# aik2mlj/polyffusion

Measured on AMD Instinct MI355X. Metric: denoising steps/sec (8-bar prmat2c, batch 16), higher is better.
Workload: dtype bf16x3; 1 GPU; sdf_chd8bar cond generation, batch 16 per GPU, 1000-step DDPM sampler loop body (BASELINE.json configs[1]); weights: deterministic synthetic, 41.08M params; global_batch=16, parallelism=batch-shard x1

## Files before the change

include/pfhip.h:

```cpp
#ifndef PFHIP_H
#define PFHIP_H

#include <stddef.h>
#include <stdint.h>

#ifdef __cplusplus
extern "C" {
#endif

#define PF_OK 0
#define PF_EINVAL (-1)
#define PF_ENOTFOUND (-2)
#define PF_ESTATE (-3)
#define PF_EHIP (-4)

int pf_version(void);
const char* pf_last_error(void);

typedef struct pf_unet pf_unet;

typedef struct pf_unet_cfg {
  int32_t in_channels, out_channels, channels, n_res_blocks;
  int32_t n_attention_levels;
  int32_t attention_levels[8];
// ... 110 lines not shown

size_t pf_packed_gemm_weight_floats(int n, int k, int taps);
int pf_pack_gemm_weight(const float* w, int n, int k, int taps, float* dst);
int pf_pack_gemm_weight_bf16x3(const float* w, int n, int k, int taps, void* dst);
int pf_pack_upfold_weight_bf16x3(const float* w, int n, int k, void* dst);
size_t pf_wino_weight_bytes(int n, int k);
int pf_pack_wino_weight_bf16x3(const float* w, int n, int k, void* dst);

int pf_gn_scale_shift(const float* x0, int c0, const float* x1, int c1, int batch, int hw, int groups, float eps,
                      const float* gamma, const float* beta, float* scale, float* shift,
                      void* scratch, size_t scratch_bytes, void* stream);
int pf_ln_stats(const float* x, int rows, int c, float eps, float* mean, float* rstd, void* stream);
int pf_ln_planes(const float* x, int rows, int c, float eps, const float* gamma, const float* beta, void* planes, void* stream);
int pf_mlp_geglu_fused(const float* x, int batch, int l, const float* ln_gamma, const float* ln_beta, float ln_eps,
                       const void* w1_bf16x3, const float* b1, const void* w2_bf16x3, const float* b2,
                       float* out, void* out_planes, void* stream);
int pf_mlp_geglu_proj_fused(const float* x, int batch, int l, const float* ln_gamma, const float* ln_beta, float ln_eps,
                            const void* w1_bf16x3, const float* b1, const void* w2_bf16x3, const float* b2,
                            const void* w3_bf16x3, const float* b3, const float* res3, float* out, float* stats3, void* stream);
typedef struct pf_conv_args {
  const float* x0; int32_t c0; const float* x1; int32_t c1;
  int32_t batch, hin, win;
  int32_t ks, stride, ups;
  const float* w; int32_t n;
  int32_t prologue; const float* sc; const float* sh; const float* mean; const float* rstd;
  const float* bias; const float* sbias; int32_t ld_sbias; const float* res; int32_t ld_res;
  int32_t geglu;
  float* out; int32_t ld_out;
  int32_t precision;
  float* stats_out;
  void* splitk_ws; size_t splitk_ws_bytes;
  int32_t a_planes;
  void* out_planes;
  void* qkv_planes;
  int32_t ups_fold;
  const float* skip_x0; int32_t skip_c0;
  const float* skip_x1; int32_t skip_c1;
  const void* skip_w;
  const float* skip_bias;
  const float* gn_stats0; int32_t gn_tiles0;
  const float* gn_stats1; int32_t gn_tiles1;
  const float* gn_gamma; const float* gn_beta;
  float gn_eps; int32_t gn_groups;
  const int64_t* sbias_rows; int32_t sbias_nrows;
  int32_t no_t16;
  int32_t no_pp;
  int32_t force_tile, force_ksplit;
  int32_t x1_bmod;
  const void* w_wino; int32_t wino;
  void* absmax_slot;
} pf_conv_args;
size_t pf_conv_splitk_ws_bytes(const pf_conv_args* a);
int pf_conv_stats_tiles(const pf_conv_args* a);
int pf_gn_finalize_tiles(const float* stats0, int tiles0, int c0, const float* stats1, int tiles1, int c1, int batch, int hw,
                         int groups, float eps, const float* gamma, const float* beta, float* scale, float* shift, void* stream);
int pf_conv2d(const pf_conv_args* a, void* stream);

int pf_attention_bf16x3(const void* qkv_planes, float* o, int ldo, void* o_planes, int batch, int n_heads, int l, int form ,
                        void* stream);
size_t pf_attention_split_scratch_bytes(int batch, int n_heads, int l);
int pf_attention_bf16x3_split(const void* qkv_planes, float* o, int ldo, void* o_planes, int batch, int n_heads, int l, void* scratch, size_t scratch_bytes,
                              void* stream);
int pf_attention(const float* q, int ldq, const float* k, int ldk, const float* v, int ldv, float* o, int ldo,
                 int batch, int n_heads, int d_head, int lq, int lk, void* stream);

typedef struct pf_ddpm pf_ddpm;
typedef struct pf_ddpm_cfg {
  int32_t image_channels, n_channels, n_levels;
  int32_t ch_mults[8];
  int32_t is_attn[8];
  int32_t n_blocks;
  int32_t img_h, img_w;
} pf_ddpm_cfg;
int pf_ddpm_create(const pf_ddpm_cfg* cfg, pf_ddpm** out);
void pf_ddpm_destroy(pf_ddpm* u);
size_t pf_ddpm_weight_bytes(const pf_ddpm* u);
int pf_ddpm_n_params(const pf_ddpm* u);
int pf_ddpm_param_info(const pf_ddpm* u, int i, char* key_buf, size_t key_buf_len, int64_t shape[4], int* ndim);
int pf_ddpm_pack_param(pf_ddpm* u, const char* key, const float* src, const int64_t* shape, int ndim, void* host_blob);
int pf_ddpm_pack_missing(const pf_ddpm* u, char* buf, size_t buf_len);
int pf_ddpm_bind_weights(pf_ddpm* u, const void* dev_blob);
int pf_ddpm_set_precision(pf_ddpm* u, int precision);
int pf_ddpm_get_precision(const pf_ddpm* u);
size_t pf_ddpm_workspace_bytes(const pf_ddpm* u, int batch);
int pf_ddpm_n_launches(const pf_ddpm* u, int batch);
double pf_ddpm_flops(const pf_ddpm* u, int batch);
int pf_ddpm_forward(pf_ddpm* u, const float* x, const int64_t* t, int batch, float* eps, void* workspace, size_t workspace_bytes, void* stream);

size_t pf_attention_wide_scratch_bytes(int batch, int l);
int pf_attention_wide(const float* q, const float* k, const float* v, int ld, float* o, int ldo, int batch, int l, int d, void* scratch,
                      size_t scratch_bytes, void* stream);
size_t pf_convt_weight_floats(int cin, int cout);
int pf_pack_convt_weight_bf16x3(const float* w, int cin, int cout, void* dst);
int pf_pack_convt_weight_f32(const float* w, int cin, int cout, float* dst);
int pf_conv_transpose_f32(const float* x, int batch, int h, int w, int cin, const float* w_packed, int cout, const float* bias, float* out,
                          void* stream);


#ifdef __cplusplus
}
#endif
#endif
```

polyffusion_amd/_lib.py:

```python
from __future__ import annotations

import ctypes as C
import os
from typing import Optional

HERE = os.path.dirname(os.path.abspath(__file__))
X3_VARIANT = {"": "", "bf16": "", "f16": "f16"}.get(os.environ.get("PF_X3", ""), None)
if X3_VARIANT is None:
    raise RuntimeError(f"PF_X3={os.environ['PF_X3']!r}: expected 'bf16' (default) or 'f16'")


def lib_path(variant: str = "") -> str:
    return os.path.join(HERE, f"libpfhip_{variant}.so" if variant else "libpfhip.so")


LIB_PATH = lib_path(X3_VARIANT)
X3_WEIGHT_SCALE = 256.0 if X3_VARIANT == "f16" else 1.0


def x3_torch_dtype(variant: Optional[str] = None):
    import torch
    return torch.float16 if (X3_VARIANT if variant is None else variant) == "f16" else torch.bfloat16


# ... 92 lines not shown
    "pf_unet_track_absmax": (C.c_int, [C.c_void_p, C.c_void_p]),
    "pf_unet_profile_read_direct": (C.c_int, [C.c_void_p, C.POINTER(C.c_double), C.c_int]),
    "pf_unet_profile_read": (C.c_int, [C.c_void_p, C.POINTER(C.c_int), c_float_p, C.POINTER(C.c_double), C.c_int]),
    "pf_unet_n_launches": (C.c_int, [C.c_void_p, C.c_int, C.c_int]),
    "pf_cfg_combine": (C.c_int, [C.c_void_p, C.c_float, C.c_void_p, C.c_size_t, C.c_void_p]),
    "pf_ddpm_step": (C.c_int, [C.c_void_p] * 6 + [C.POINTER(DdpmCoef), C.c_void_p, C.c_size_t, C.c_void_p]),
    "pf_axpby": (C.c_int, [C.c_void_p, C.c_void_p, C.c_float, C.c_float, C.c_void_p, C.c_size_t, C.c_void_p]),
    "pf_ddim_step": (C.c_int, [C.c_void_p] * 6 + [C.POINTER(DdimCoef), C.c_void_p, C.c_size_t, C.c_void_p]),
    "pf_randn": (C.c_int, [C.c_void_p, C.c_size_t, C.c_uint64, C.c_uint64, C.c_uint64, C.c_void_p]),
    "pf_ddpm_step_rng": (C.c_int, [C.c_void_p] * 4 + [C.POINTER(DdpmCoef), C.c_uint64, C.c_uint64, C.c_uint64, C.c_uint64, C.c_void_p, C.c_size_t, C.c_void_p]),
    "pf_ddim_step_rng": (C.c_int, [C.c_void_p] * 5 + [C.POINTER(DdimCoef), C.c_uint64, C.c_uint64, C.c_uint64, C.c_void_p, C.c_size_t, C.c_void_p]),
    "pf_ddpm_step_rng_dev": (C.c_int, [C.c_void_p] * 6 + [C.c_uint64, C.c_uint64, C.c_void_p, C.c_size_t, C.c_void_p]),
    "pf_ddim_step_rng_dev": (C.c_int, [C.c_void_p] * 7 + [C.c_uint64, C.c_uint64, C.c_void_p, C.c_size_t, C.c_void_p]),
    "pf_clock_probe": (C.c_int, [C.c_void_p, C.c_void_p]),
    "pf_mfma_probe": (C.c_int, [C.c_void_p, C.c_int, C.POINTER(C.c_double), C.c_void_p]),
    "pf_step_state_set": (C.c_int, [C.c_void_p, C.c_int64, C.c_uint64, C.c_void_p]),
    "pf_step_begin": (C.c_int, [C.c_void_p, C.c_void_p, C.c_void_p, C.c_int, C.c_void_p]),
    "pf_step_end": (C.c_int, [C.c_void_p, C.c_int, C.c_void_p]),
    "pf_randn_dev": (C.c_int, [C.c_void_p, C.c_size_t, C.c_uint64, C.c_void_p, C.c_int, C.c_uint64, C.c_void_p]),
    "pf_ddpm_step_dev": (C.c_int, [C.c_void_p] * 6 + [C.c_void_p, C.c_void_p, C.c_void_p, C.c_size_t, C.c_void_p]),
    "pf_ddim_step_dev": (C.c_int, [C.c_void_p] * 6 + [C.c_void_p, C.c_void_p, C.c_void_p, C.c_size_t, C.c_void_p]),
    "pf_comm_unique_id": (C.c_int, [C.c_void_p]),
    "pf_comm_init": (C.c_int, [C.c_void_p, C.c_int, C.c_int, C.POINTER(C.c_void_p)]),
    "pf_comm_bcast": (C.c_int, [C.c_void_p, C.c_void_p, C.c_size_t, C.c_int, C.c_void_p]),
    "pf_comm_destroy": (C.c_int, [C.c_void_p]),
    "pf_prmat2c_durations": (C.c_int, [C.c_void_p, C.c_int, C.c_int, C.c_int, C.c_void_p, C.c_void_p]),
    "pf_encoder_create": (C.c_int, [C.c_int] * 6 + [C.POINTER(C.c_void_p)]),
    "pf_encoder_destroy": (None, [C.c_void_p]),
    "pf_encoder_weight_bytes": (C.c_size_t, [C.c_void_p]),
    "pf_encoder_pack_param": (C.c_int, [C.c_void_p, C.c_char_p, C.c_void_p, c_i64_p, C.c_int, C.c_void_p]),
    "pf_encoder_pack_missing": (C.c_int, [C.c_void_p, C.c_char_p, C.c_size_t]),
    "pf_encoder_bind_weights": (C.c_int, [C.c_void_p, C.c_void_p]),
    "pf_encoder_workspace_bytes": (C.c_size_t, [C.c_void_p, C.c_int]),
    "pf_encoder_forward": (C.c_int, [C.c_void_p, C.c_void_p, C.c_int, C.c_int, C.c_void_p, C.c_void_p, C.c_size_t, C.c_void_p]),
    "pf_packed_gemm_weight_floats": (C.c_size_t, [C.c_int, C.c_int, C.c_int]),
    "pf_pack_gemm_weight": (C.c_int, [C.c_void_p, C.c_int, C.c_int, C.c_int, C.c_void_p]),
    "pf_pack_gemm_weight_bf16x3": (C.c_int, [C.c_void_p, C.c_int, C.c_int, C.c_int, C.c_void_p]),
    "pf_pack_upfold_weight_bf16x3": (C.c_int, [C.c_void_p, C.c_int, C.c_int, C.c_void_p]),
    "pf_wino_weight_bytes": (C.c_size_t, [C.c_int, C.c_int]),
    "pf_pack_wino_weight_bf16x3": (C.c_int, [C.c_void_p, C.c_int, C.c_int, C.c_void_p]),
    "pf_unet_set_precision": (C.c_int, [C.c_void_p, C.c_int]),
    "pf_unet_get_precision": (C.c_int, [C.c_void_p]),
    "pf_x3_element": (C.c_int, []),
    "pf_gn_scale_shift": (C.c_int, [C.c_void_p, C.c_int, C.c_void_p, C.c_int, C.c_int, C.c_int, C.c_int, C.c_float,
                                    C.c_void_p, C.c_void_p, C.c_void_p, C.c_void_p, C.c_void_p, C.c_size_t, C.c_void_p]),
    "pf_ln_stats": (C.c_int, [C.c_void_p, C.c_int, C.c_int, C.c_float, C.c_void_p, C.c_void_p, C.c_void_p]),
    "pf_ln_planes": (C.c_int, [C.c_void_p, C.c_int, C.c_int, C.c_float, C.c_void_p, C.c_void_p, C.c_void_p, C.c_void_p]),
    "pf_mlp_geglu_fused": (C.c_int, [C.c_void_p, C.c_int, C.c_int, C.c_void_p, C.c_void_p, C.c_float, C.c_void_p, C.c_void_p, C.c_void_p,
                                     C.c_void_p, C.c_void_p, C.c_void_p, C.c_void_p]),
    "pf_mlp_geglu_proj_fused": (C.c_int, [C.c_void_p, C.c_int, C.c_int, C.c_void_p, C.c_void_p, C.c_float] + [C.c_void_p] * 10),
    "pf_conv2d": (C.c_int, [C.POINTER(ConvArgs), C.c_void_p]),
    "pf_conv_stats_tiles": (C.c_int, [C.POINTER(ConvArgs)]),
    "pf_conv_splitk_ws_bytes": (C.c_size_t, [C.POINTER(ConvArgs)]),
    "pf_gn_finalize_tiles": (C.c_int, [C.c_void_p, C.c_int, C.c_int, C.c_void_p, C.c_int, C.c_int, C.c_int, C.c_int, C.c_int,
                                       C.c_float, C.c_void_p, C.c_void_p, C.c_void_p, C.c_void_p, C.c_void_p]),
    "pf_attention_bf16x3": (C.c_int, [C.c_void_p, C.c_void_p, C.c_int, C.c_void_p, C.c_int, C.c_int, C.c_int, C.c_int, C.c_void_p]),
    "pf_attention_split_scratch_bytes": (C.c_size_t, [C.c_int, C.c_int, C.c_int]),
    "pf_attention_bf16x3_split": (C.c_int, [C.c_void_p, C.c_void_p, C.c_int, C.c_void_p, C.c_int, C.c_int, C.c_int, C.c_void_p, C.c_size_t, C.c_void_p]),
    "pf_attention": (C.c_int, [C.c_void_p, C.c_int, C.c_void_p, C.c_int, C.c_void_p, C.c_int, C.c_void_p, C.c_int,
                               C.c_int, C.c_int, C.c_int, C.c_int, C.c_int, C.c_void_p]),
    "pf_ddpm_create": (C.c_int, [C.POINTER(DDPMCfg), C.POINTER(C.c_void_p)]),
    "pf_ddpm_destroy": (None, [C.c_void_p]),
    "pf_ddpm_weight_bytes": (C.c_size_t, [C.c_void_p]),
    "pf_ddpm_n_params": (C.c_int, [C.c_void_p]),
    "pf_ddpm_param_info": (C.c_int, [C.c_void_p, C.c_int, C.c_char_p, C.c_size_t, c_i64_p, C.POINTER(C.c_int)]),
    "pf_ddpm_pack_param": (C.c_int, [C.c_void_p, C.c_char_p, C.c_void_p, c_i64_p, C.c_int, C.c_void_p]),
    "pf_ddpm_pack_missing": (C.c_int, [C.c_void_p, C.c_char_p, C.c_size_t]),
    "pf_ddpm_bind_weights": (C.c_int, [C.c_void_p, C.c_void_p]),
    "pf_ddpm_set_precision": (C.c_int, [C.c_void_p, C.c_int]),
    "pf_ddpm_get_precision": (C.c_int, [C.c_void_p]),
    "pf_ddpm_workspace_bytes": (C.c_size_t, [C.c_void_p, C.c_int]),
    "pf_ddpm_n_launches": (C.c_int, [C.c_void_p, C.c_int]),
    "pf_ddpm_flops": (C.c_double, [C.c_void_p, C.c_int]),
    "pf_ddpm_forward": (C.c_int, [C.c_void_p, C.c_void_p, C.c_void_p, C.c_int, C.c_void_p, C.c_void_p, C.c_size_t, C.c_void_p]),
    "pf_attention_wide_scratch_bytes": (C.c_size_t, [C.c_int, C.c_int]),
    "pf_attention_wide": (C.c_int, [C.c_void_p, C.c_void_p, C.c_void_p, C.c_int, C.c_void_p, C.c_int, C.c_int, C.c_int, C.c_int,
                                    C.c_void_p, C.c_size_t, C.c_void_p]),
    "pf_convt_weight_floats": (C.c_size_t, [C.c_int, C.c_int]),
    "pf_pack_convt_weight_bf16x3": (C.c_int, [C.c_void_p, C.c_int, C.c_int, C.c_void_p]),
    "pf_pack_convt_weight_f32": (C.c_int, [C.c_void_p, C.c_int, C.c_int, C.c_void_p]),
    "pf_conv_transpose_f32": (C.c_int, [C.c_void_p, C.c_int, C.c_int, C.c_int, C.c_int, C.c_void_p, C.c_int, C.c_void_p, C.c_void_p,
                                        C.c_void_p]),
}

_libs: dict = {}


def load(variant: Optional[str] = None) -> C.CDLL:
    v = X3_VARIANT if variant is None else variant
    if v in _libs:
        return _libs[v]
    path = lib_path(v)
    if not os.path.exists(path):
        raise RuntimeError(
            f"{path} not found: the HIP extension is not built. Run `python -m polyffusion_amd.build{' --variant=' + v if v else ''}` "
            "(or __graft_entry__.build()). There is no CPU fallback for this path.")
    lib = C.CDLL(path, mode=os.RTLD_LOCAL | os.RTLD_NOW)
    for name, (res, args) in SIGNATURES.items():
        fn = getattr(lib, name)
        fn.restype = res
        fn.argtypes = args
    if lib.pf_x3_element() != (1 if v == "f16" else 0):
        raise RuntimeError(f"{path}: built with the wrong split element type (pf_x3_element() = {lib.pf_x3_element()})")
    _libs[v] = lib
    return lib

# ... 22 lines not shown
```

polyffusion_amd/build.py:

```python
from __future__ import annotations

import os
import subprocess
import sys

HERE = os.path.dirname(os.path.abspath(__file__))
CSRC = os.path.join(HERE, "csrc")
SOURCES = ["conv_mfma.hip", "conv_bf16x3.hip", "conv_wino.hip", "gemm_planes_bf3.hip", "mlp_fused_bf3.hip", "attention.hip", "attention_bf3.hip", "norm_stats.hip", "small_kernels.hip", "encoders.hip", "comm.hip", "plan.hip", "unet_blocks.hip", "unet.hip", "attention_wide.hip", "ddpm_unet.hip", "abi_ops.hip"]
LIB = os.path.join(HERE, "libpfhip.so")
VARIANTS = {"": [], "f16": ["-DPF_X3_F16"]}


def lib_path(variant: str = "") -> str:
    return os.path.join(HERE, f"libpfhip_{variant}.so" if variant else "libpfhip.so")
HIPCC = os.environ.get("HIPCC", "/opt/rocm/bin/hipcc")
FLAGS = ["--offload-arch=gfx950", "-O3", "-std=c++17", "-fPIC", "-Wall", "-Wno-unused-function"] + (["-DPF_TRACE"] if os.environ.get("PF_TRACE") else [])
EXTRA_FLAGS = {"attention_bf3.hip": ["-fno-slp-vectorize"]}


STAMP = os.path.join(CSRC, ".build_stamp.json")


def _digest(paths, extra=()) -> str:
    import hashlib
    h = hashlib.sha256()
    for p in paths:
        with open(p, "rb") as f:
            h.update(hashlib.sha256(f.read()).digest())
    for e in extra:
        h.update(str(e).encode())
        h.update(b"\0")
    return h.hexdigest()


def _read_stamp() -> dict:
    import json
    try:
        with open(STAMP) as f:
            return json.load(f)
    except (OSError, ValueError):
        return {}


def _write_stamp(st: dict) -> None:
    import json
    with open(STAMP + ".new", "w") as f:
        json.dump(st, f, indent=1, sort_keys=True)
    os.replace(STAMP + ".new", STAMP)


def build(force: bool = False, verbose: bool = True, variant: str = "") -> str:
    return build_all(force, verbose, (variant,))[0]


_SLOW_FIRST = ["conv_bf16x3.hip", "conv_wino.hip", "attention_bf3.hip", "mlp_fused_bf3.hip", "conv_mfma.hip", "gemm_planes_bf3.hip"]


def build_all(force: bool = False, verbose: bool = True, variants=("", "f16")) -> list:
    force = force or os.environ.get("PF_FORCE_BUILD", "") not in ("", "0")
    hdrs = [os.path.join(CSRC, h) for h in sorted(os.listdir(CSRC)) if h.endswith(".h")] + [os.path.join(HERE, "..", "include", "pfhip.h")]
    stamp = _read_stamp()
# ... 49 lines not shown
```

polyffusion_amd/csrc/abi_ops.hip:

```cpp
#include <stdarg.h>
#include <vector>
#include "plan.h"

namespace pf {

static thread_local std::string g_err;
int set_error(int code, const char* fmt, ...) {
  char buf[512];
  va_list ap;
  va_start(ap, fmt);
  vsnprintf(buf, sizeof buf, fmt, ap);
  va_end(ap);
  g_err = buf;
  return code;
}

}

using namespace pf;

extern "C" {

int pf_version(void) { return 100; }
const char* pf_last_error(void) { return g_err.c_str(); }
// ... 9 lines not shown
int pf_pack_gemm_weight(const float* w, int n, int k, int taps, float* dst) {
  PF_REQUIRE(w && dst && n > 0 && k > 0 && k % 4 == 0 && (taps == 1 || taps == 9), "pf_pack_gemm_weight: bad arguments");
  memset(dst, 0, gemm_floats(taps, k, n) * sizeof(float));
  pack_gemm(dst, w, n, k, taps, (n + 63) / 64 * 64, 0);
  return PF_OK;
}

int pf_pack_gemm_weight_bf16x3(const float* w, int n, int k, int taps, void* dst) {
  PF_REQUIRE(w && dst && n > 0 && k > 0 && k % 8 == 0 && (taps == 1 || taps == 9), "pf_pack_gemm_weight_bf16x3: bad arguments");
  memset(dst, 0, gemm_floats(taps, k, n) * sizeof(float));
  PF_REQUIRE(pack_gemm_bf3(dst, w, n, k, taps, (n + 63) / 64 * 64, 0, nullptr), X3_RANGE_MSG, "pf_pack_gemm_weight_bf16x3");
  return PF_OK;
}

int pf_gn_scale_shift(const float* x0, int c0, const float* x1, int c1, int batch, int hw, int groups, float eps,
                      const float* gamma, const float* beta, float* scale, float* shift, void* scratch, size_t scratch_bytes,
                      void* stream) {
  return launch_gn_scale_shift(x0, c0, x1, c1, batch, hw, groups, eps, gamma, beta, scale, shift, scratch, scratch_bytes, (hipStream_t)stream);
}
int pf_pack_upfold_weight_bf16x3(const float* w, int n, int k, void* dst) {
  PF_REQUIRE(w && dst && n > 0 && k > 0 && k % 8 == 0, "pack_upfold: bad arguments");
  PF_REQUIRE(pack_upfold_bf3(dst, w, n, k, (n + 63) / 64 * 64), X3_RANGE_MSG, "pf_pack_upfold_weight_bf16x3");
  return PF_OK;
}
size_t pf_wino_weight_bytes(int n, int k) { return (n > 0 && k > 0) ? (size_t)16 * k * n * 4 : 0; }
int pf_pack_wino_weight_bf16x3(const float* w, int n, int k, void* dst) {
  PF_REQUIRE(w && dst && n > 0 && k > 0 && n % 64 == 0 && k % 16 == 0, "pack_wino: n must be a multiple of 64 and k of 16 (n=%d k=%d)", n, k);
  PF_REQUIRE(pack_wino_bf3(dst, w, n, k), X3_RANGE_MSG, "pf_pack_wino_weight_bf16x3");
  return PF_OK;
}
int pf_prmat2c_durations(const float* prmat2c, int n, int steps, int custom_round, int32_t* dur, void* stream) {
  return launch_prmat2c_durations(prmat2c, n, steps, custom_round, dur, (hipStream_t)stream);
}
int pf_mlp_geglu_fused(const float* x, int batch, int l, const float* ln_gamma, const float* ln_beta, float ln_eps,
                       const void* w1_bf16x3, const float* b1, const void* w2_bf16x3, const float* b2,
                       float* out, void* out_planes, void* stream) {
  return launch_mlp_fused(x, batch, l, ln_gamma, ln_beta, ln_eps, w1_bf16x3, b1, w2_bf16x3, b2, out, out_planes, (hipStream_t)stream);
}
int pf_mlp_geglu_proj_fused(const float* x, int batch, int l, const float* ln_gamma, const float* ln_beta, float ln_eps,
                            const void* w1_bf16x3, const float* b1, const void* w2_bf16x3, const float* b2,
                            const void* w3_bf16x3, const float* b3, const float* res3, float* out, float* stats3, void* stream) {
  if (!w3_bf16x3) return set_error(PF_EINVAL, "pf_mlp_geglu_proj_fused: null projection weight");
  return launch_mlp_fused(x, batch, l, ln_gamma, ln_beta, ln_eps, w1_bf16x3, b1, w2_bf16x3, b2, out, nullptr, (hipStream_t)stream, w3_bf16x3, b3,
                          res3, stats3);
}
int pf_ln_planes(const float* x, int rows, int c, float eps, const float* gamma, const float* beta, void* planes, void* stream) {
  return launch_ln_planes(x, rows, c, eps, gamma, beta, planes, (hipStream_t)stream);
}
int pf_ln_stats(const float* x, int rows, int c, float eps, float* mean, float* rstd, void* stream) {
  return launch_ln_stats(x, rows, c, eps, mean, rstd, (hipStream_t)stream);
}
int pf_conv_stats_tiles(const pf_conv_args* a) { return a ? conv_stats_tiles(*a) : 0; }
size_t pf_conv_splitk_ws_bytes(const pf_conv_args* a) { return a ? conv_splitk_ws_bytes(*a) : 0; }
int pf_gn_finalize_tiles(const float* stats0, int tiles0, int c0, const float* stats1, int tiles1, int c1, int batch, int hw,
                         int groups, float eps, const float* gamma, const float* beta, float* scale, float* shift, void* stream) {
  return launch_gn_finalize_tiles(stats0, tiles0, c0, stats1, tiles1, c1, batch, hw, groups, eps, gamma, beta, scale, shift,
                                  (hipStream_t)stream);
}
int pf_conv2d(const pf_conv_args* a, void* stream) {
  PF_REQUIRE(a, "pf_conv2d: null argument");
  return launch_conv(*a, (hipStream_t)stream);
}
size_t pf_attention_split_scratch_bytes(int batch, int n_heads, int l) {
  return (batch > 0 && n_heads > 0 && l > 0) ? attention_bf3_split_floats(batch, n_heads, l, nullptr) * sizeof(float) : 0;
}
int pf_attention_bf16x3_split(const void* qkv_planes, float* o, int ldo, void* o_planes, int batch, int n_heads, int l, void* scratch, size_t scratch_bytes,
                              void* stream) {
  return launch_attention_bf3(qkv_planes, o, ldo, o_planes, batch, n_heads, l, 0, (hipStream_t)stream, static_cast<float*>(scratch), scratch_bytes / sizeof(float));
}
int pf_attention_bf16x3(const void* qkv_planes, float* o, int ldo, void* o_planes, int batch, int n_heads, int l, int form, void* stream) {
  return launch_attention_bf3(qkv_planes, o, ldo, o_planes, batch, n_heads, l, form, (hipStream_t)stream);
}
int pf_attention(const float* q, int ldq, const float* k, int ldk, const float* v, int ldv, float* o, int ldo, int batch,
                 int n_heads, int d_head, int lq, int lk, void* stream) {
  PF_REQUIRE(q && k && v && o, "pf_attention: null argument");
  return launch_attention(q, ldq, k, ldk, v, ldv, o, ldo, batch, n_heads, d_head, lq, lk, (hipStream_t)stream);
}

int pf_cfg_combine(const float* eps2, float scale, float* eps, size_t n, void* stream) { return launch_cfg_combine(eps2, scale, eps, n, (hipStream_t)stream); }
int pf_ddpm_step(const float* x, const float* eps, const float* noise_p, const float* noise_q, const float* orig, const float* mask,
                 const pf_ddpm_coef* c, float* x_out, size_t n, void* stream) {
  PF_REQUIRE(c, "pf_ddpm_step: null coefficients");
  return launch_ddpm_step(x, eps, noise_p, noise_q, orig, mask, *c, x_out, n, (hipStream_t)stream);
}
int pf_axpby(const float* x, const float* noise, float a, float b, float* out, size_t n, void* stream) { return launch_axpby(x, noise, a, b, out, n, (hipStream_t)stream); }
int pf_ddim_step(const float* x, const float* eps, const float* noise, const float* orig, const float* orig_noise, const float* mask,
                 const pf_ddim_coef* c, float* x_out, size_t n, void* stream) {
  PF_REQUIRE(c, "pf_ddim_step: null coefficients");
  return launch_ddim_step(x, eps, noise, orig, orig_noise, mask, *c, x_out, n, (hipStream_t)stream);
}
int pf_randn(float* out, size_t n, uint64_t seed, uint64_t stream_id, uint64_t elem_offset, void* stream) {
  return launch_randn(out, n, seed, stream_id, elem_offset, (hipStream_t)stream);
}
int pf_ddpm_step_rng(const float* x, const float* eps, const float* orig, const float* mask, const pf_ddpm_coef* c, uint64_t seed,
                     uint64_t draw_q, uint64_t draw_p, uint64_t elem_offset, float* x_out, size_t n, void* stream) {
  PF_REQUIRE(c, "pf_ddpm_step_rng: null coefficients");
  return launch_ddpm_step_rng(x, eps, orig, mask, c, nullptr, nullptr, seed, draw_q, draw_p, elem_offset, x_out, n, (hipStream_t)stream);
}
int pf_ddim_step_rng(const float* x, const float* eps, const float* orig, const float* orig_noise, const float* mask, const pf_ddim_coef* c,
                     uint64_t seed, uint64_t draw, uint64_t elem_offset, float* x_out, size_t n, void* stream) {
  PF_REQUIRE(c, "pf_ddim_step_rng: null coefficients");
  return launch_ddim_step_rng(x, eps, orig, orig_noise, mask, c, nullptr, nullptr, seed, draw, elem_offset, x_out, n, (hipStream_t)stream);
}
int pf_ddpm_step_rng_dev(const float* x, const float* eps, const float* orig, const float* mask, const pf_ddpm_coef* table,
                         const pf_step_state* st, uint64_t seed, uint64_t elem_offset, float* x_out, size_t n, void* stream) {
  PF_REQUIRE(table && st, "pf_ddpm_step_rng_dev: null table / state");
// ... 54 lines not shown
```

polyffusion_amd/csrc/conv_bf16x3.hip:

```cpp
#include <vector>

#include "conv_common.h"

namespace pf {

#ifdef PF_TRACE
__device__ unsigned long long g_trace[8192];
#define TR() do { if (trace_on && tslot < 2040) { g_trace[tbase + tslot++] = __builtin_amdgcn_s_memtime(); } } while (0)
#else
#define TR() do {} while (0)
#endif

typedef x3_t x3x4 __attribute__((ext_vector_type(4)));

template <int KS, int STRIDE, int TWIN, int BN>
constexpr int conv_bf3_row_pitch() {
  return (KS != 1 && STRIDE == 1 && BN >= 128) ? (TWIN * 40 + 127) / 128 * 128 : TWIN * 40;
}

#ifndef PF_KG2_RING
#define PF_KG2_RING 5
#endif
template <int KS, int BN, int KG>
constexpr bool conv_bf3_pingpong() { return KS == 3 && BN == 128 && KG == 2; }
// ... 732 lines not shown
  constexpr int FMFN = (TH * TW / NWM / 32) * (BN / 2 / 32);
  constexpr size_t lds_groups = KG * conv_bf3_group_lds<KS, STRIDE, TH, TW, BN, SKIP, KG>();
  constexpr size_t lds_xch = KG == 2 ? (size_t)FMFN * 16 * NWM * 128 * 4 : 0;
  constexpr size_t lds = lds_groups > lds_xch ? lds_groups : lds_xch;
  static_assert(lds <= 160 * 1024, "LDS budget");
  p.tiles_x = cdiv(p.Wout, TW);
  p.tiles_y = cdiv(p.Hout, TH);
  p.nt = cdiv(p.Npad, BN);
  conv_fill_divs(p);
  auto kern = conv_bf3_kernel<KS, STRIDE, UPS, TH, TW, BN, PRO, NWM, SKIP, KG>;
  static std::atomic<uint64_t> attr_done{0};
  if (int rc = set_max_lds_once(reinterpret_cast<const void*>(kern), (int)lds, attr_done)) return rc;
  const int grid = p.B * p.tiles_y * p.tiles_x * p.nt * p.ksplit * (KS == 2 ? 4 : 1);
  hipLaunchKernelGGL(kern, dim3(grid), dim3(KG * NWM * 128), lds, stream, p);
  PF_CHECK_HIP(hipGetLastError());
  return PF_OK;
}

template <int KS, int STRIDE, bool UPS, int PRO>
static int dispatch_tile3(ConvP& p, int tile, hipStream_t s) {
  if constexpr (KS == 1) {
    if (tile == 0) return launch3_cfg<1, 1, false, 1, 128, 128, PRO>(p, s);
    if (tile == 1) return launch3_cfg<1, 1, false, 1, 128, 64, PRO>(p, s);
    return launch3_cfg<1, 1, false, 1, 64, 64, PRO>(p, s);
  } else if constexpr (KS == 2) {
    if (tile == 0) return launch3_cfg<2, 1, false, 8, 16, 128, PRO>(p, s);
    if (tile == 1) return launch3_cfg<2, 1, false, 8, 16, 64, PRO>(p, s);
    return launch3_cfg<2, 1, false, 4, 16, 64, PRO>(p, s);
  } else if constexpr (STRIDE == 2) {
    return launch3_cfg<3, 2, false, 4, 16, 64, PRO>(p, s);
  } else {
    if constexpr (!UPS && PRO == 1) {
      const int blocks = p.B * cdiv(p.Hout, tile == 3 ? 16 : tile == 2 ? 4 : 8) * cdiv(p.Wout, 16) * cdiv(p.Npad, tile == 0 ? 128 : 64);
      const int cus = num_cus();
      const bool kg2 = tile == 2 && p.ksplit == 1 && blocks <= cus && ((p.c0 + p.c1) / 32) % 2 == 0 && (!p.sw || ((p.sc0 + p.sc1) / 32) % 2 == 0);
      if (kg2) return p.sw ? launch3_cfg<3, 1, false, 4, 16, 64, 1, 2, true, 2>(p, s) : launch3_cfg<3, 1, false, 4, 16, 64, 1, 2, false, 2>(p, s);
      if (p.pp && tile == 0 && p.ksplit == 1 && blocks <= cus && (p.c0 + p.c1) >= 256 && ((p.c0 + p.c1) / 32) % 2 == 0 && (!p.sw || ((p.sc0 + p.sc1) / 32) % 2 == 0))
        return p.sw ? launch3_cfg<3, 1, false, 8, 16, 128, 1, 2, true, 2>(p, s) : launch3_cfg<3, 1, false, 8, 16, 128, 1, 2, false, 2>(p, s);
      if (tile == 3) return p.sw ? launch3_cfg<3, 1, false, 16, 16, 64, 1, 2, true>(p, s) : launch3_cfg<3, 1, false, 16, 16, 64, 1, 2, false>(p, s);
      if (p.sw) {
        if (tile == 0) return launch3_cfg<3, 1, false, 8, 16, 128, 1, 2, true>(p, s);
        if (tile == 1) return launch3_cfg<3, 1, false, 8, 16, 64, 1, 2, true>(p, s);
        return launch3_cfg<3, 1, false, 4, 16, 64, 1, 2, true>(p, s);
      }
    }
    if (tile == 0) return launch3_cfg<3, 1, UPS, 8, 16, 128, PRO>(p, s);
    if (tile == 1) return launch3_cfg<3, 1, UPS, 8, 16, 64, PRO>(p, s);
    return launch3_cfg<3, 1, UPS, 4, 16, 64, PRO>(p, s);
  }
}

int launch_conv_bf3(const pf_conv_args& a, hipStream_t stream) {
  if (conv_wino_eligible(a)) return launch_conv_wino(a, stream);
  ConvP p;
  memset(&p, 0, sizeof p);
  p.x0 = a.x0; p.x1 = a.x1; p.c0 = a.c0; p.c1 = a.c1;
  p.B = a.batch; p.Hin = a.hin; p.Win = a.win;
  p.Hout = a.hin; p.Wout = a.win;
  if (a.ups) { p.Hout *= 2; p.Wout *= 2; }
  if (a.stride == 2) { p.Hout = (p.Hout - 1) / 2 + 1; p.Wout = (p.Wout - 1) / 2 + 1; }
  p.w = a.w; p.N = a.n; p.Npad = (a.n + 63) / 64 * 64;
  p.sc = a.sc; p.sh = a.sh; p.mean = a.mean; p.rstd = a.rstd;
  p.bias = a.bias; p.sbias = a.sbias; p.ld_sbias = a.ld_sbias; p.res = a.res; p.ld_res = a.ld_res;
  p.sb_rows = reinterpret_cast<const long long*>(a.sbias_rows); p.sb_nrows = a.sbias_nrows;
  p.geglu = a.geglu; p.out = a.out; p.ld_out = a.ld_out; p.stats = a.stats_out;
  p.ksplit = conv_ksplit(a);
  p.pp = !a.no_pp;
  p.partial = p.ksplit > 1 ? static_cast<float*>(a.splitk_ws) : nullptr;
  p.qkv = a.qkv_planes; p.out_planes = a.out_planes;
  if (a.gn_stats0 && (a.prologue == 1 || a.prologue == 2)) {
    p.gn_s0 = a.gn_stats0; p.gn_t0 = a.gn_tiles0; p.gn_s1 = a.gn_stats1; p.gn_t1 = a.gn_tiles1;
    p.gn_gamma = a.gn_gamma; p.gn_beta = a.gn_beta; p.gn_eps = a.gn_eps; p.gn_groups = a.gn_groups;
  }
  p.sx0 = a.skip_x0; p.sc0 = a.skip_c0; p.sx1 = a.skip_x1; p.sc1 = a.skip_c1; p.sw = a.skip_w; p.bias2 = a.skip_w ? a.skip_bias : nullptr;
  p.x1_bmod = a.x1_bmod;
  p.amax = static_cast<unsigned*>(a.absmax_slot);
  const int tile = conv_pick_tile(a);
  if (a.ks == 1) {
    switch (a.prologue) {
      case 0: return dispatch_tile3<1, 1, false, 0>(p, tile, stream);
      case 2: return dispatch_tile3<1, 1, false, 2>(p, tile, stream);
      default: return dispatch_tile3<1, 1, false, 3>(p, tile, stream);
    }
  }
  if (a.ups_fold) {
    p.Hout = a.hin; p.Wout = a.win; p.fold = 1;
    return dispatch_tile3<2, 1, false, 0>(p, tile, stream);
  }
  if (a.stride == 2) return dispatch_tile3<3, 2, false, 0>(p, tile, stream);
  int rc = a.ups ? dispatch_tile3<3, 1, true, 0>(p, tile, stream) : dispatch_tile3<3, 1, false, 1>(p, tile, stream);
  if (rc != PF_OK || p.ksplit == 1) return rc;
  const int M = p.B * p.Hout * p.Wout;
  hipLaunchKernelGGL(splitk_reduce_kernel, dim3(M / 64, cdiv(p.N, 64)), dim3(1024), 0, stream, static_cast<const float*>(a.splitk_ws), p.ksplit, M, p.N,
                     p.Hout * p.Wout, p.bias, p.bias2, p.sbias, p.ld_sbias, p.sb_rows, p.sb_nrows, p.res, p.ld_res, p.out, p.ld_out, p.stats, p.amax);
  PF_CHECK_HIP(hipGetLastError());
  return PF_OK;
}

#ifdef PF_TRACE
extern "C" int pf_debug_trace_read(unsigned long long* dst, int n) {
  return hipMemcpyFromSymbol(dst, HIP_SYMBOL(g_trace), (size_t)n * 8) == hipSuccess ? 0 : -1;
}
extern "C" int pf_debug_trace_clear() {
  static unsigned long long z[8192];
  return hipMemcpyToSymbol(HIP_SYMBOL(g_trace), z, sizeof z) == hipSuccess ? 0 : -1;
}
// ... 57 lines not shown
```

polyffusion_amd/csrc/pf_internal.h:

```cpp
#pragma once
#include <hip/hip_runtime.h>
#include <stdint.h>
#include <stdio.h>
#include <string.h>
#include <atomic>
#include <string>
#include "../../include/pfhip.h"

typedef float f32x16 __attribute__((ext_vector_type(16)));
typedef float f32x4 __attribute__((ext_vector_type(4)));

namespace pf {

int set_error(int code, const char* fmt, ...);

#define PF_CHECK_HIP(expr)                                                                   \
  do {                                                                                       \
    hipError_t _e = (expr);                                                                  \
    if (_e != hipSuccess) return pf::set_error(PF_EHIP, "%s: %s", #expr, hipGetErrorString(_e)); \
  } while (0)

#define PF_REQUIRE(cond, ...)                                   \
  do {                                                          \
    if (!(cond)) return pf::set_error(PF_EINVAL, __VA_ARGS__);  \
  } while (0)

static inline int cdiv(int a, int b) { return (a + b - 1) / b; }

static inline int set_max_lds_once(const void* kern, int bytes, std::atomic<uint64_t>& done_mask) {
  int dev = 0;
  PF_CHECK_HIP(hipGetDevice(&dev));
  const uint64_t bit = 1ull << (dev & 63);
  if (done_mask.load(std::memory_order_acquire) & bit) return PF_OK;
  PF_CHECK_HIP(hipFuncSetAttribute(kern, hipFuncAttributeMaxDynamicSharedMemorySize, bytes));
  done_mask.fetch_or(bit, std::memory_order_release);
  return PF_OK;
}
int num_cus();
static inline size_t align_up(size_t v, size_t a) { return (v + a - 1) / a * a; }

int launch_conv(const pf_conv_args& a, hipStream_t stream);
double conv_flops(const pf_conv_args& a);
int launch_conv_bf3(const pf_conv_args& a, hipStream_t stream);
int conv_pick_tile(const pf_conv_args& a);
void conv_tile_shape(const pf_conv_args& a, int tile, int* th, int* tw);
int conv_stats_tiles(const pf_conv_args& a);
int conv_ksplit(const pf_conv_args& a);
size_t conv_splitk_ws_bytes(const pf_conv_args& a);
bool pack_gemm_bf3(void* dst, const float* src, int n_src, int K, int taps, int Npad, int n_off, const int* colmap);
bool pack_upfold_bf3(void* dst, const float* src, int N, int K, int Npad);
bool conv_wino_eligible(const pf_conv_args& a);
int launch_conv_wino(const pf_conv_args& a, hipStream_t stream);
bool pack_wino_bf3(void* dst, const float* src, int N, int K);

int launch_attention(const float* q, int ldq, const float* k, int ldk, const float* v, int ldv, float* o, int ldo,
                     int batch, int n_heads, int d_head, int lq, int lk, hipStream_t stream);

int launch_attention_bf3(const void* planes, float* o, int ldo, void* o_planes, int batch, int n_heads, int l, int form, hipStream_t stream,
                         float* scratch = nullptr, size_t scratch_floats = 0);
size_t attention_bf3_split_floats(int batch, int n_heads, int l, int* nsplit_out);
int launch_gemm_planes(const pf_conv_args& a, hipStream_t stream);
int launch_mlp_fused(const float* x, int batch, int l, const float* gamma, const float* beta, float eps, const void* w1, const float* b1,
                     const void* w2, const float* b2, float* out, void* out_planes, hipStream_t stream, const void* w3 = nullptr,
                     const float* b3 = nullptr, const float* res3 = nullptr, float* stats3 = nullptr);

size_t gn_scratch_bytes(int batch, int c, int hw);
int launch_gn_scale_shift(const float* x0, int c0, const float* x1, int c1, int batch, int hw, int groups, float eps,
                          const float* gamma, const float* beta, float* scale, float* shift, void* scratch,
                          size_t scratch_bytes, hipStream_t stream);
int launch_gn_finalize_tiles(const float* s0, int t0, int c0, const float* s1, int t1, int c1, int batch, int hw, int groups,
                             float eps, const float* gamma, const float* beta, float* scale, float* shift, hipStream_t stream, int bmod1 = 0);
int gn_nsplit(int hw);
int launch_gn_partial(const float* x0, int c0, const float* x1, int c1, int batch, int hw, float* stats, hipStream_t stream);
int launch_ln_stats(const float* x, int rows, int c, float eps, float* mean, float* rstd, hipStream_t stream);
int launch_ln_planes(const float* x, int rows, int c, float eps, const float* gamma, const float* beta, void* planes,
                     hipStream_t stream);

int launch_conv_in(const float* x_nchw, const float* w , const float* bias, float* out_nhwc,
                   int batch, int cin, int cout, int h, int w_, hipStream_t stream, float* stats = nullptr);
int launch_conv_in_stats_tiles(int cin, int cout, int h, int w_);
int launch_conv_out(const float* x_nhwc, const float* sc, const float* sh, const float* w ,
                    const float* bias, float* out_nchw, int batch, int cin, int cout, int h, int w_, hipStream_t stream);

int launch_time_embed(const int64_t* t, const float* w0, const float* b0, const float* w2, const float* b2,
                      float* out_silu, int batch, int channels, int d_t, hipStream_t stream);
int launch_prmat2c_durations(const float* x, int n, int steps, int custom_round, int32_t* dur, hipStream_t stream);
int launch_matvec(const float* x, int ldx, const float* w, const float* bias, float* y, int ldy, int batch, int n, int k,
                  hipStream_t stream, int n_per_group = 0, int x_group_stride = 0);

int launch_cfg_combine(const float* eps2, float scale, float* eps, size_t n, hipStream_t s);
int launch_ddpm_step(const float* x, const float* eps, const float* noise_p, const float* noise_q, const float* orig,
                     const float* mask, const pf_ddpm_coef& c, float* out, size_t n, hipStream_t s);
int launch_axpby(const float* x, const float* y, float a, float b, float* out, size_t n, hipStream_t s);
int launch_ddim_step(const float* x, const float* eps, const float* noise, const float* orig, const float* orig_noise,
                     const float* mask, const pf_ddim_coef& c, float* out, size_t n, hipStream_t s);
int launch_randn(float* out, size_t n, uint64_t seed, uint64_t stream_id, uint64_t elem_offset, hipStream_t s);
int launch_randn_dev(float* out, size_t n, uint64_t seed, const pf_step_state* st, int slot, uint64_t elem_offset, hipStream_t s);
int launch_ddpm_step_dev(const float* x, const float* eps, const float* noise_p, const float* noise_q, const float* orig,
                         const float* mask, const pf_ddpm_coef* table, const pf_step_state* st, float* out, size_t n, hipStream_t s);
int launch_ddim_step_dev(const float* x, const float* eps, const float* noise, const float* orig, const float* orig_noise,
                         const float* mask, const pf_ddim_coef* table, const pf_step_state* st, float* out, size_t n, hipStream_t s);
int launch_ddpm_step_rng(const float* x, const float* eps, const float* orig, const float* mask, const pf_ddpm_coef* c_host,
                         const pf_ddpm_coef* table, const pf_step_state* st, uint64_t seed, uint64_t draw_q, uint64_t draw_p, uint64_t off,
                         float* out, size_t n, hipStream_t s);
int launch_ddim_step_rng(const float* x, const float* eps, const float* orig, const float* orig_noise, const float* mask,
// ... 51 lines not shown
```

Before: 206.9 steps/s.

## Add row-form 1x1 conv kernel with register-ring weights for bf16x3

```diff
diff --git a/include/pfhip.h b/include/pfhip.h
--- a/include/pfhip.h
+++ b/include/pfhip.h
@@ -186,6 +186,7 @@
 } pf_conv_args;
 size_t pf_conv_splitk_ws_bytes(const pf_conv_args* a);
 int pf_conv_stats_tiles(const pf_conv_args* a);
+int pf_conv_row_form_eligible(const pf_conv_args* a);
 int pf_gn_finalize_tiles(const float* stats0, int tiles0, int c0, const float* stats1, int tiles1, int c1, int batch, int hw,
                          int groups, float eps, const float* gamma, const float* beta, float* scale, float* shift, void* stream);
 int pf_conv2d(const pf_conv_args* a, void* stream);
diff --git a/polyffusion_amd/_lib.py b/polyffusion_amd/_lib.py
--- a/polyffusion_amd/_lib.py
+++ b/polyffusion_amd/_lib.py
@@ -168,6 +168,7 @@
     "pf_conv2d": (C.c_int, [C.POINTER(ConvArgs), C.c_void_p]),
     "pf_conv_stats_tiles": (C.c_int, [C.POINTER(ConvArgs)]),
     "pf_conv_splitk_ws_bytes": (C.c_size_t, [C.POINTER(ConvArgs)]),
+    "pf_conv_row_form_eligible": (C.c_int, [C.POINTER(ConvArgs)]),
     "pf_gn_finalize_tiles": (C.c_int, [C.c_void_p, C.c_int, C.c_int, C.c_void_p, C.c_int, C.c_int, C.c_int, C.c_int, C.c_int,
                                        C.c_float, C.c_void_p, C.c_void_p, C.c_void_p, C.c_void_p, C.c_void_p]),
     "pf_attention_bf16x3": (C.c_int, [C.c_void_p, C.c_void_p, C.c_int, C.c_void_p, C.c_int, C.c_int, C.c_int, C.c_int, C.c_void_p]),
diff --git a/polyffusion_amd/build.py b/polyffusion_amd/build.py
--- a/polyffusion_amd/build.py
+++ b/polyffusion_amd/build.py
@@ -6,7 +6,7 @@
 
 HERE = os.path.dirname(os.path.abspath(__file__))
 CSRC = os.path.join(HERE, "csrc")
-SOURCES = ["conv_mfma.hip", "conv_bf16x3.hip", "conv_wino.hip", "gemm_planes_bf3.hip", "mlp_fused_bf3.hip", "attention.hip", "attention_bf3.hip", "norm_stats.hip", "small_kernels.hip", "encoders.hip", "comm.hip", "plan.hip", "unet_blocks.hip", "unet.hip", "attention_wide.hip", "ddpm_unet.hip", "abi_ops.hip"]
+SOURCES = ["conv_mfma.hip", "conv_bf16x3.hip", "conv_wino.hip", "conv1x1_rows_bf3.hip", "gemm_planes_bf3.hip", "mlp_fused_bf3.hip", "attention.hip", "attention_bf3.hip", "norm_stats.hip", "small_kernels.hip", "encoders.hip", "comm.hip", "plan.hip", "unet_blocks.hip", "unet.hip", "attention_wide.hip", "ddpm_unet.hip", "abi_ops.hip"]
 LIB = os.path.join(HERE, "libpfhip.so")
 VARIANTS = {"": [], "f16": ["-DPF_X3_F16"]}
 
diff --git a/polyffusion_amd/csrc/abi_ops.hip b/polyffusion_amd/csrc/abi_ops.hip
--- a/polyffusion_amd/csrc/abi_ops.hip
+++ b/polyffusion_amd/csrc/abi_ops.hip
@@ -85,6 +85,7 @@
 }
 int pf_conv_stats_tiles(const pf_conv_args* a) { return a ? conv_stats_tiles(*a) : 0; }
 size_t pf_conv_splitk_ws_bytes(const pf_conv_args* a) { return a ? conv_splitk_ws_bytes(*a) : 0; }
+int pf_conv_row_form_eligible(const pf_conv_args* a) { return a && conv_rows_tile(*a) ? 1 : 0; }
 int pf_gn_finalize_tiles(const float* stats0, int tiles0, int c0, const float* stats1, int tiles1, int c1, int batch, int hw,
                          int groups, float eps, const float* gamma, const float* beta, float* scale, float* shift, void* stream) {
   return launch_gn_finalize_tiles(stats0, tiles0, c0, stats1, tiles1, c1, batch, hw, groups, eps, gamma, beta, scale, shift,
diff --git a/polyffusion_amd/csrc/conv1x1_rows_bf3.hip b/polyffusion_amd/csrc/conv1x1_rows_bf3.hip
--- /dev/null
+++ b/polyffusion_amd/csrc/conv1x1_rows_bf3.hip
@@ -0,0 +1,207 @@
+#include "conv_common.h"
+
+namespace pf {
+
+typedef x3_t x3x4 __attribute__((ext_vector_type(4)));
+
+#ifdef PF_TRACE
+__device__ unsigned long long g_rows_trace[16];
+#define RTR(i) do { if (trace_on) { __builtin_amdgcn_sched_barrier(0); tstamp[i] = __builtin_amdgcn_s_memtime(); __builtin_amdgcn_sched_barrier(0); } } while (0)
+#else
+#define RTR(i) do {} while (0)
+#endif
+
+struct RowsP {
+  ConvP c;
+  int pro;
+};
+
+constexpr int ROWS_KMAX = 256;
+
+static size_t rows_lds_bytes(int bm, int k) { return (size_t)2 * bm * (k + 8) * sizeof(x3_t); }
+
+template <int BM, int FN, int NCH>
+__global__ __launch_bounds__(256, 2) void conv1x1_rows_kernel(RowsP rp) {
+  constexpr int FM = BM / 32;
+  constexpr int K = NCH * 32, TPR = K / 4, RPP = 256 / TPR;
+  constexpr int NA = (BM + RPP - 1) / RPP;
+  constexpr int RING = 3;
+  const ConvP& p = rp.c;
+  extern __shared__ __attribute__((aligned(16))) unsigned char smem[];
+  const int tid = threadIdx.x, lane = tid & 63;
+  const int wave = __builtin_amdgcn_readfirstlane(tid >> 6);
+#ifdef PF_TRACE
+  const bool trace_on = threadIdx.x == 0 && (blockIdx.x == 0 || blockIdx.x == gridDim.x - 1);
+  unsigned long long tstamp[8];
+#endif
+  RTR(0);
+  const int b = fdiv(blockIdx.x, p.d_tx), r0 = (blockIdx.x - b * p.tiles_x) * BM;
+  const int L = p.Wout;
+  constexpr int pitch = K + 8;
+  x3_t* sAh = reinterpret_cast<x3_t*>(smem);
+  x3_t* sAl = sAh + BM * pitch;
+
+  const x3_t* wl = static_cast<const x3_t*>(p.w) + ((lane >> 5) * 2 * p.Npad + wave * (32 * FN) + (lane & 31)) * 8;
+  const int wplane = p.Npad * 8, wstep = 4 * wplane;
+  u32x4 wr[RING][2][2][FN];
+  auto loadW = [&](int chunk, auto slot) {
+#pragma unroll
+    for (int s = 0; s < 2; ++s)
+#pragma unroll
+      for (int pl = 0; pl < 2; ++pl)
+#pragma unroll
+        for (int fn = 0; fn < FN; ++fn)
+          wr[slot.value][s][pl][fn] = *reinterpret_cast<const u32x4*>(wl + (chunk * 2 + s) * wstep + pl * wplane + fn * 256);
+  };
+
+  const int arow = tid / TPR, c4 = tid % TPR;
+  const bool aact = arow < RPP;
+  const float* xb = p.x0 + (size_t)b * L * K;
+  f32x4 ra[NA];
+#pragma unroll
+  for (int i = 0; i < NA; ++i)
+    ra[i] = *reinterpret_cast<const f32x4*>(xb + min(r0 + min(arow + i * RPP, BM - 1), L - 1) * K + c4 * 4);
+  loadW(0, std::integral_constant<int, 0>{});
+  if constexpr (NCH > 1) loadW(1, std::integral_constant<int, 1>{});
+  __builtin_amdgcn_sched_barrier(0);
+  RTR(1);
+
+  f32x4 vsc = {1.f, 1.f, 1.f, 1.f}, vsh = {0.f, 0.f, 0.f, 0.f};
+  if (rp.pro) {
+    if (p.gn_s0) gn_fused_prologue<256>(p, b, tid, p.Hin * p.Win, reinterpret_cast<double*>(smem));
+    vsc = *reinterpret_cast<const f32x4*>(p.sc + (size_t)b * K + c4 * 4);
+    vsh = *reinterpret_cast<const f32x4*>(p.sh + (size_t)b * K + c4 * 4);
+  }
+  RTR(2);
+#pragma unroll
+  for (int i = 0; i < NA; ++i) {
+    const int row = arow + i * RPP;
+    if (aact && row < BM) {
+      f32x4 v = ra[i];
+      if (rp.pro) v = v * vsc + vsh;
+      const x3x4 qh = __builtin_convertvector(v, x3x4);
+      const f32x4 hf = __builtin_convertvector(qh, f32x4);
+      const x3x4 ql = __builtin_convertvector(v - hf, x3x4);
+      *reinterpret_cast<x3x4*>(sAh + row * pitch + c4 * 4) = qh;
+      *reinterpret_cast<x3x4*>(sAl + row * pitch + c4 * 4) = ql;
+    }
+  }
+  RTR(3);
+  __syncthreads();
+  RTR(4);
+
+  f32x16 acc[FM][FN];
+#pragma unroll
+  for (int fm = 0; fm < FM; ++fm)
+#pragma unroll
+    for (int fn = 0; fn < FN; ++fn)
+#pragma unroll
+      for (int r = 0; r < 16; ++r) acc[fm][fn][r] = 0.f;
+  const x3_t* aH = sAh + (lane & 31) * pitch + 8 * (lane >> 5);
+  const x3_t* aL = sAl + (lane & 31) * pitch + 8 * (lane >> 5);
+  static_for<0, NCH>([&](auto cc) {
+    constexpr int c = decltype(cc)::value;
+    {
+      __builtin_amdgcn_sched_barrier(0);
+      if constexpr (c + 2 < NCH) loadW(c + 2, std::integral_constant<int, (c + 2) % RING>{});
+      __builtin_amdgcn_sched_barrier(0);
+#pragma unroll
+      for (int s = 0; s < 2; ++s) {
+        x3x8 ah[FM], al[FM];
+#pragma unroll
+        for (int fm = 0; fm < FM; ++fm) {
+          ah[fm] = *reinterpret_cast<const x3x8*>(aH + fm * 32 * pitch + c * 32 + s * 16);
+          al[fm] = *reinterpret_cast<const x3x8*>(aL + fm * 32 * pitch + c * 32 + s * 16);
+        }
+#pragma unroll
+        for (int fm = 0; fm < FM; ++fm)
+#pragma unroll
+          for (int fn = 0; fn < FN; ++fn) acc[fm][fn] = x3_mfma_32x32x16(al[fm], __builtin_bit_cast(x3x8, wr[c % RING][s][0][fn]), acc[fm][fn], 0, 0, 0);
+#pragma unroll
+        for (int fm = 0; fm < FM; ++fm)
+#pragma unroll
+          for (int fn = 0; fn < FN; ++fn) acc[fm][fn] = x3_mfma_32x32x16(ah[fm], __builtin_bit_cast(x3x8, wr[c % RING][s][1][fn]), acc[fm][fn], 0, 0, 0);
+#pragma unroll
+        for (int fm = 0; fm < FM; ++fm)
+#pragma unroll
+          for (int fn = 0; fn < FN; ++fn) acc[fm][fn] = x3_mfma_32x32x16(ah[fm], __builtin_bit_cast(x3x8, wr[c % RING][s][0][fn]), acc[fm][fn], 0, 0, 0);
+      }
+    }
+  });
+
+  RTR(5);
+  x3_unscale(acc);
+  conv_epilogue<1, BM, 64 * FN, FM, FN, 1>(p, acc, b, 0, r0, (wave >> 1) * (64 * FN), 0, wave & 1, lane, tid, reinterpret_cast<float*>(smem));
+#ifdef PF_TRACE
+  asm volatile("s_waitcnt vmcnt(0)" ::: "memory");
+  RTR(6);
+  if (trace_on)
+    for (int i = 0; i < 7; ++i) g_rows_trace[(blockIdx.x == 0 ? 0 : 8) + i] = tstamp[i];
+#endif
+}
+
+static int rows_pick_bm(int batch, long long L) { return (long long)batch * ((L + 63) / 64) >= num_cus() ? 64 : 32; }
+
+int conv_rows_tile(const pf_conv_args& a) {
+  if (a.precision != PF_PREC_BF16X3 || a.ks != 1 || a.stride != 1 || a.ups || a.ups_fold || (a.prologue != 0 && a.prologue != 2)) return 0;
+  if (a.c1 != 0 || a.a_planes || a.geglu || a.qkv_planes || a.out_planes || a.stats_out || a.res || a.sbias || a.skip_w) return 0;
+  if (a.force_tile) return 0;
+  if (a.n % 128 != 0 || a.n > 256 || a.c0 % 32 != 0 || a.c0 > ROWS_KMAX) return 0;
+  if (a.ld_out < a.n || a.batch <= 0 || a.hin <= 0 || a.win <= 0) return 0;
+  const long long L = (long long)a.hin * a.win;
+  if (L * a.c0 >= (1ll << 31) || L * a.ld_out >= (1ll << 31) || (long long)a.batch * ((L + 31) / 32) >= (1ll << 31)) return 0;
+  const int bm = rows_pick_bm(a.batch, L);
+  return rows_lds_bytes(bm, a.c0) <= 80 * 1024 ? bm : 0;
+}
+
+template <int BM, int FN, int NCH>
+static int launch_rows_cfg(RowsP& rp, hipStream_t stream) {
+  ConvP& p = rp.c;
+  p.tiles_x = cdiv(p.Wout, BM); p.tiles_y = 1; p.nt = 1;
+  conv_fill_divs(p);
+  const size_t lds = rows_lds_bytes(BM, NCH * 32);
+  auto kern = conv1x1_rows_kernel<BM, FN, NCH>;
+  static std::atomic<uint64_t> attr_done{0};
+  if (int rc = set_max_lds_once(reinterpret_cast<const void*>(kern), (int)lds, attr_done)) return rc;
+  hipLaunchKernelGGL(kern, dim3(p.B * p.tiles_x), dim3(256), lds, stream, rp);
+  PF_CHECK_HIP(hipGetLastError());
+  return PF_OK;
+}
+
+template <int NCH>
+static int launch_rows_k(RowsP& rp, int nch, int bm, int fn, hipStream_t stream) {
+  if constexpr (NCH > ROWS_KMAX / 32) return -1;
+  else {
+    if (nch != NCH) return launch_rows_k<NCH + 1>(rp, nch, bm, fn, stream);
+    if (bm == 64) return fn == 2 ? launch_rows_cfg<64, 2, NCH>(rp, stream) : launch_rows_cfg<64, 1, NCH>(rp, stream);
+    return fn == 2 ? launch_rows_cfg<32, 2, NCH>(rp, stream) : launch_rows_cfg<32, 1, NCH>(rp, stream);
+  }
+}
+
+#ifdef PF_TRACE
+extern "C" int pf_debug_rows_trace_read(unsigned long long* dst) {
+  return hipMemcpyFromSymbol(dst, HIP_SYMBOL(g_rows_trace), sizeof(unsigned long long) * 16) == hipSuccess ? 0 : -1;
+}
+#endif
+
+int launch_conv_rows(const pf_conv_args& a, hipStream_t stream) {
+  RowsP rp;
+  memset(&rp, 0, sizeof rp);
+  ConvP& p = rp.c;
+  p.x0 = a.x0; p.c0 = a.c0;
+  p.B = a.batch; p.Hin = 1; p.Win = a.hin * a.win; p.Hout = 1; p.Wout = p.Win;
+  p.w = a.w; p.N = a.n; p.Npad = (a.n + 63) / 64 * 64;
+  p.sc = a.sc; p.sh = a.sh; p.bias = a.bias; p.out = a.out; p.ld_out = a.ld_out;
+  p.ksplit = 1;
+  if (a.gn_stats0 && a.prologue == 2) {
+    p.gn_s0 = a.gn_stats0; p.gn_t0 = a.gn_tiles0;
+    p.gn_gamma = a.gn_gamma; p.gn_beta = a.gn_beta; p.gn_eps = a.gn_eps; p.gn_groups = a.gn_groups;
+  }
+  p.amax = static_cast<unsigned*>(a.absmax_slot);
+  rp.pro = a.prologue;
+  const int bm = conv_rows_tile(a), fn = a.n / 128;
+  const int rc = launch_rows_k<1>(rp, a.c0 / 32, bm, fn, stream);
+  return rc >= 0 ? rc : set_error(PF_EINVAL, "conv: no row form for these arguments");
+}
+
+}
diff --git a/polyffusion_amd/csrc/conv_bf16x3.hip b/polyffusion_amd/csrc/conv_bf16x3.hip
--- a/polyffusion_amd/csrc/conv_bf16x3.hip
+++ b/polyffusion_amd/csrc/conv_bf16x3.hip
@@ -808,6 +808,7 @@
 
 int launch_conv_bf3(const pf_conv_args& a, hipStream_t stream) {
   if (conv_wino_eligible(a)) return launch_conv_wino(a, stream);
+  if (conv_rows_tile(a)) return launch_conv_rows(a, stream);
   ConvP p;
   memset(&p, 0, sizeof p);
   p.x0 = a.x0; p.x1 = a.x1; p.c0 = a.c0; p.c1 = a.c1;
diff --git a/polyffusion_amd/csrc/pf_internal.h b/polyffusion_amd/csrc/pf_internal.h
--- a/polyffusion_amd/csrc/pf_internal.h
+++ b/polyffusion_amd/csrc/pf_internal.h
@@ -51,6 +51,8 @@
 bool pack_upfold_bf3(void* dst, const float* src, int N, int K, int Npad);
 bool conv_wino_eligible(const pf_conv_args& a);
 int launch_conv_wino(const pf_conv_args& a, hipStream_t stream);
+int conv_rows_tile(const pf_conv_args& a);
+int launch_conv_rows(const pf_conv_args& a, hipStream_t stream);
 bool pack_wino_bf3(void* dst, const float* src, int N, int K);
 
 int launch_attention(const float* q, int ldq, const float* k, int ldk, const float* v, int ldv, float* o, int ldo,
```

Measured after the change: 208.1 steps/s (median of 6 runs). About the same (+0.6%).
